# wwang2/CoarseGrainingVAE

Hardware: AMD Instinct MI355X
Metric: train_step_frames_per_sec (higher is better)
Workload: dtype f32

## Files before the change

coarsegrainingvae_amd/_lib.py:

```python
from __future__ import annotations

import ctypes as C
import os
import re
import threading

import torch

from . import ktimer

_PKG = os.path.dirname(os.path.abspath(__file__))
LIB_PATH = os.environ.get("CGV_LIB") or os.path.join(_PKG, "libcgvae_hip.so")
HEADER_PATH = os.path.join(os.path.dirname(_PKG), "include", "cgvae_hip.h")

_lock = threading.Lock()
_lib = None

_p, _i, _f, _sz = C.c_void_p, C.c_int, C.c_float, C.c_size_t

PROTOTYPES = {
    "cgv_version": (_i, []),
    "cgv_last_error_string": (C.c_char_p, []),
    "cgv_timestamp": (_i, [_p, _p]),
    "cgv_timestamp_hz": (_i, []),
# ... 93 lines not shown
    "cgv_decoder_slices_to_dense": (_i, [_p, _p, _i, C.c_int64, _p, _i, _i, _p]),
    "cgv_dense_grad_prepare": (_i, [_p, _p, _p, _p, _i, _i, _i, _i, _p]),
    "cgv_tile_supported": (_i, [_i, _i, _i]),
    "cgv_tile_linear_fwd": (_i, [_p, _p, _p, _p, _p, _i, _i, _i, _i, _p]),
    "cgv_tile_linear_bwd_input": (_i, [_p, _p, _p, _i, _i, _i, _p]),
    "cgv_tile_linear_bwd_input_act": (_i, [_p, _p, _p, _p, _i, _i, _i, _i, _p]),
    "cgv_tile_linear_bwd_input_act_add": (_i, [_p, _p, _p, _p, _p, _i, _i, _i, _i, _p]),
    "cgv_tile_linear_bwd_input_act_add_bcast": (_i, [_p] * 7 + [_i, _p, _i, _i, _i, _i, _p]),
    "cgv_tile_pair_supported": (_i, [_i, _i, _i]),
    "cgv_tile_pair_linear_fwd": (_i, [_p] * 10 + [_i, _i, _i, _i, _i, _p]),
    "cgv_tile_pair_linear_bwd_input": (_i, [_p] * 10 + [_i, _i, _i, _i, _i, _p]),
    "cgv_tile_linear_bwd_input_out": (_i, [_p] * 5 + [_i, _i, _i, _i, _p, _i, _p]),
    "cgv_tile_bwd_input_split": (_i, [_p, _sz, _p]),
    "cgv_tile_pair_linear_bwd_input_out": (_i, [_p] * 10 + [_i, _i, _i, _i, _i, _p, _i, _p, _i, _p]),
    "cgv_tile_linear_bwd_input_sum2": (_i, [_p] * 10 + [_i, _p, _i, _i, _i, _i, _i, _p]),
    "cgv_segment_reduce2": (_i, [_p, _i, _p, _p, _i, _p, _p, _p, _i, _i, _p]),
    "cgv_skinny_linear_bwd_input_add": (_i, [_p, _p, _p, _p, _p, _i, _i, _i, _i, _p, _sz, _p]),
    "cgv_skinny_linear_bwd_input_out": (_i, [_p] * 5 + [_i, _i, _i, _i, _p, _i, _p, _sz, _p]),
    "cgv_tile_linear_wgrad": (_i, [_p, _p, _p, _i, _i, _i, _i, _p]),
    "cgv_wgrad_record_bytes": (_i, []),
    "cgv_wgrad_plan": (_i, [_i, _i, _i, _p, _p, _p]),
    "cgv_wgrad_lds_floats": (_i, [_i, _i]),
    "cgv_grouped_wgrad": (_i, [_p, _i, _i, _i, _p]),
    "cgv_wgrad_gathered_plan": (_i, [_i, _i, _i, _i, _p, _p]),
    "cgv_grouped_wgrad_gathered": (_i, [_p, _i, _i, _p]),
    "cgv_wgrad_gathered_plan_tile": (_i, [_i, _i, _i, _i, _i, _p, _p]),
    "cgv_grouped_wgrad_gathered_tile": (_i, [_p, _i, _i, _i, _p]),
    "cgv_grouped_wgrad_split": (_i, [_p, _i, _i, _p]),
    "cgv_grouped_wgrad_gathered_sumsq": (_i, [_p, _i, _i, _p, _p, _p]),
    "cgv_grouped_wgrad_gathered_adam": (_i, [_p, _i, _i, _p, _p, _p, _p, _f, _f, _f, _f, _p, _p]),
# ... 236 lines not shown
```

coarsegrainingvae_amd/csrc/tile_gemm.hip:

```cpp
#include <stdlib.h>
#include <initializer_list>
#include <type_traits>
#include "cgv_common.h"
#include "streamk_gemm.h"

namespace cgv {

typedef float f32x4 __attribute__((ext_vector_type(4)));

__device__ __forceinline__ float4 ld4z(const float* p, bool ok) {
  return ok ? *reinterpret_cast<const float4*>(p) : make_float4(0.f, 0.f, 0.f, 0.f);
}

#define CGV_MFMA(a, b, c) __builtin_amdgcn_mfma_f32_16x16x4f32((a), (b), (c), 0, 0, 0)

template <int I0, int N, typename F>
__device__ __forceinline__ void static_for(F&& f) {
  if constexpr (I0 < N) {
    f(std::integral_constant<int, I0>{});
    static_for<I0 + 1, N>(f);
  }
}

struct TileSecond { const float* x; const float* W; const float* bias; float* y; float* z; int act; };
// ... 366 lines not shown
      float4 zv = make_float4(acc[a][b][0] + bv.x, acc[a][b][1] + bv.y, acc[a][b][2] + bv.z, acc[a][b][3] + bv.w);
      if (act) {
        if (zout) *reinterpret_cast<float4*>(zout + (size_t)m * N + n) = zv;
        zv.x = act_fwd(zv.x, act); zv.y = act_fwd(zv.y, act); zv.z = act_fwd(zv.z, act); zv.w = act_fwd(zv.w, act);
      }
      *reinterpret_cast<float4*>(y + (size_t)m * N + n) = zv;
    }
  }
}

struct BwdSource { const float* g; const float* W; const float* z; int act; };
struct BwdSecond { const float* g; const float* W; float* gx; const float* z; const float* add; int act; };
struct OutAct { const float* z; int act; const float* z2; int act2; };
struct SplitN { float* part; unsigned* ticket; int n; };
struct NormStackOut { const float* stack; const float* Vv; const float* g_res; float* g_s; float* gVv; int F; int ld; int accumulate; };
struct BcastAdd {
  const float* src;
  const int64_t* row2seg;
  const int* rowptr;
  int mean;
};

#ifndef CGV_BWD_INPUT_PIPELINE
#define CGV_BWD_INPUT_PIPELINE 0
#endif
template <int MB, int WAVES>
__global__ __launch_bounds__(64 * WAVES) void tile_bwd_input_k(const float* __restrict__ g, const float* __restrict__ W,
                                                        float* __restrict__ gx, int M, int N, int K,
                                                        const float* __restrict__ z, int act,
                                                        const float* __restrict__ add = nullptr,
                                                        BcastAdd bc = BcastAdd{nullptr, nullptr, nullptr, 0},
                                                        BwdSecond s2 = BwdSecond{nullptr, nullptr, nullptr, nullptr, nullptr, 0},
                                                        BwdSource more = BwdSource{nullptr, nullptr, nullptr, 0},
                                                        OutAct oa = OutAct{nullptr, 0, nullptr, 0},
                                                        SplitN sp = SplitN{nullptr, nullptr, 1},
                                                        NormStackOut ns = NormStackOut{nullptr, nullptr, nullptr, nullptr, nullptr, 0, 0, 0}) {
  if (blockIdx.z) { g = s2.g; W = s2.W; gx = s2.gx; z = s2.z; add = s2.add; act = s2.act; bc.src = nullptr; oa.z = oa.z2; oa.act = oa.act2; }
  __shared__ float red[WAVES][MB * 4][4][64];
  const int lane = threadIdx.x & 63;
  const int wave = __builtin_amdgcn_readfirstlane(threadIdx.x >> 6);
  const int j = lane & 15, q = lane >> 4;
  const int ry = (int)blockIdx.y / sp.n, zs = (int)blockIdx.y - ry * sp.n;
  const int k0 = blockIdx.x * 64, m0 = ry * (16 * MB);
  const int kcol = k0 + 4 * j;
  const bool kok = kcol < K;
  const float* gr[MB];
  bool gok[MB];
#pragma unroll
  for (int mb = 0; mb < MB; ++mb) {
    const int m = m0 + 16 * mb + j;
    gok[mb] = m < M;
    gr[mb] = g + (size_t)(gok[mb] ? m : 0) * N + 4 * q;
  }
  const ptrdiff_t zoff = act ? z - g : 0;
  f32x4 acc[MB][4];
#pragma unroll
  for (int mb = 0; mb < MB; ++mb)
#pragma unroll
    for (int s = 0; s < 4; ++s) acc[mb][s] = f32x4{0.f, 0.f, 0.f, 0.f};
  const int steps_all = (N + 15) / 16, zper = (steps_all + sp.n - 1) / sp.n;
  const int z_beg = min(zs * zper, steps_all), steps = min(z_beg + zper, steps_all);
  const int per = (steps - z_beg + WAVES - 1) / WAVES;
  const int st_beg = min(z_beg + wave * per, steps), st_end = min(st_beg + per, steps);
  constexpr int SB = WAVES >= 16 ? 3 : 2;
  const float* wcol = W + (kok ? kcol : 0);
  ptrdiff_t zo = zoff;
  const int n_src = more.g ? 2 : 1;
  for (int src = 0; src < n_src; ++src) {
  if (src == 1) {
#pragma unroll
    for (int mb = 0; mb < MB; ++mb) gr[mb] = more.g + (gr[mb] - g);
    act = more.act;
    zo = act ? more.z - more.g : 0;
    wcol = more.W + (kok ? kcol : 0);
  }
  struct Batch { float4 a[SB][MB], zz[SB][MB], b[SB][4]; };
  auto request = [&](Batch& B, int st0) __attribute__((always_inline)) {
#pragma unroll
    for (int u = 0; u < SB; ++u) {
      const int n = 16 * (st0 + u);
      const bool in = st0 + u < st_end && n + 4 * q < N;
      const int ng = in ? n : -4 * q, nw = in ? n + 4 * q : 0;
#pragma unroll
      for (int mb = 0; mb < MB; ++mb) {
        B.a[u][mb] = *reinterpret_cast<const float4*>(gr[mb] + ng);
        if (act) B.zz[u][mb] = *reinterpret_cast<const float4*>(gr[mb] + zo + ng);
      }
#pragma unroll
      for (int c = 0; c < 4; ++c) B.b[u][c] = *reinterpret_cast<const float4*>(wcol + (size_t)(nw + c) * K);
    }
  };
  auto multiply = [&](const Batch& B, int st0) __attribute__((always_inline)) {
#pragma unroll
    for (int u = 0; u < SB; ++u) {
      if (st0 + u >= st_end) break;
      const bool nok = 16 * (st0 + u) + 4 * q < N;
#pragma unroll
      for (int mb = 0; mb < MB; ++mb) {
        float4 av = B.a[u][mb];
        if (act) {
          av.x *= act_bwd(B.zz[u][mb].x, act); av.y *= act_bwd(B.zz[u][mb].y, act);
          av.z *= act_bwd(B.zz[u][mb].z, act); av.w *= act_bwd(B.zz[u][mb].w, act);
        }
        const float ac[4] = {nok ? av.x : 0.f, nok ? av.y : 0.f, nok ? av.z : 0.f, nok ? av.w : 0.f};
#pragma unroll
        for (int c = 0; c < 4; ++c) {
          acc[mb][0] = CGV_MFMA(ac[c], B.b[u][c].x, acc[mb][0]);
          acc[mb][1] = CGV_MFMA(ac[c], B.b[u][c].y, acc[mb][1]);
          acc[mb][2] = CGV_MFMA(ac[c], B.b[u][c].z, acc[mb][2]);
          acc[mb][3] = CGV_MFMA(ac[c], B.b[u][c].w, acc[mb][3]);
        }
// ... 335 lines not shown
  const int blocks16 = kt * ((M + 15) / 16);
  const int ow = option(CGV_OPT_BWD_INPUT_WAVES);
  int waves = 8;
  if (ow > 0 && ow != 32) waves = ow;
  else if (blocks16 < 128 && N >= 1024) waves = 16;
  if (ow == 32 || (blocks32 >= 200 && blocks32 < 512 && waves == 8))
    c.kernel = BWD_R32_W8;
  else if (blocks32 >= 512)
    c.kernel = BWD_R32_W4;
  else if (waves == 16) {
    c.kernel = BWD_R16_W16;
    if (ws) c.shares = split_shares(blocks16 * np, N);
  }
  return c;
}
}

static int tile_bwd_input_launch(const float* g, const float* z, int act, const float* W, float* gx, int M, int N, int K,
                                 void* stream, const char* what, const float* add = nullptr,
                                 cgv::BcastAdd bc = cgv::BcastAdd{nullptr, nullptr, nullptr, 0},
                                 const cgv::BwdSecond* second = nullptr,
                                 cgv::BwdSource more = cgv::BwdSource{nullptr, nullptr, nullptr, 0},
                                 cgv::OutAct oa = cgv::OutAct{nullptr, 0, nullptr, 0},
                                 cgv::NormStackOut ns = cgv::NormStackOut{nullptr, nullptr, nullptr, nullptr, nullptr, 0, 0, 0}) {
  hipStream_t st = (hipStream_t)stream;
  const cgv::BwdSecond s2 = second ? *second : cgv::BwdSecond{nullptr, nullptr, nullptr, nullptr, nullptr, 0};
  const unsigned np = second ? 2u : 1u;
  const cgv::BwdInputChoice choice = cgv::bwd_input_choice(M, N, K, (int)np, cgv::sk_ws_ready(stream));
  if (const int bpc = choice.bpc;
      bpc != 0 && !ns.stack && act == 0 && (!more.g || more.act == 0) && (!second || s2.act == 0) &&
      cgv::sk_aligned({g, W, gx, add, bc.src, more.g, more.W, oa.z, oa.z2, s2.g, s2.W, s2.gx, s2.add})) {
    cgv::SkArgs a{};
    a.np = (int)np; a.M = M; a.N = K;
    cgv::SkProblem& p0 = a.p[0];
    p0.A[0] = g; p0.B[0] = W; p0.R[0] = N; p0.out = gx; p0.add = add;
    if (more.g) { p0.A[1] = more.g; p0.B[1] = more.W; p0.R[1] = N; }
    p0.bc_src = bc.src; p0.bc_row2seg = bc.row2seg; p0.bc_rowptr = bc.rowptr; p0.bc_mean = bc.mean;
    p0.oz = oa.z; p0.oact = oa.act;
    if (second) {
      cgv::SkProblem& p1 = a.p[1];
      p1.A[0] = s2.g; p1.B[0] = s2.W; p1.R[0] = N; p1.out = s2.gx; p1.add = s2.add; p1.oz = oa.z2; p1.oact = oa.act2;
    }
    if (cgv::sk_launch(a, true, cgv::g_split_ws.ws, cgv::g_split_ws.bytes, cgv::SPLIT_TICKET_BYTES, st, bpc) == 0)
      return cgv::check_launch(what);
  }
  const int kt = (K + 63) / 64;
  switch (choice.kernel) {
    case cgv::BWD_R32_W8:
      hipLaunchKernelGGL((cgv::tile_bwd_input_k<2, 8>), dim3(kt, (M + 31) / 32, np), dim3(512), 0, st, g, W, gx, M, N, K, z, act, add, bc, s2, more, oa, cgv::SplitN{nullptr, nullptr, 1}, ns);
      break;
    case cgv::BWD_R32_W4:
      hipLaunchKernelGGL((cgv::tile_bwd_input_k<2, 4>), dim3(kt, (M + 31) / 32, np), dim3(256), 0, st, g, W, gx, M, N, K, z, act, add, bc, s2, more, oa, cgv::SplitN{nullptr, nullptr, 1}, ns);
      break;
    case cgv::BWD_R16_W16: {
      cgv::SplitN sp{nullptr, nullptr, 1};
      const int tiles = kt * ((M + 15) / 16) * (int)np;
      const cgv::SplitWs& w = cgv::g_split_ws;
      const size_t need = cgv::SPLIT_TICKET_BYTES + (size_t)tiles * choice.shares * (16 * 64) * sizeof(float);
      if (choice.shares > 1 && need <= w.bytes && (size_t)tiles * sizeof(unsigned) <= cgv::SPLIT_TICKET_BYTES) {
        sp.ticket = reinterpret_cast<unsigned*>(w.ws);
        sp.part = reinterpret_cast<float*>(reinterpret_cast<char*>(w.ws) + cgv::SPLIT_TICKET_BYTES);
        sp.n = choice.shares;
      }
      hipLaunchKernelGGL((cgv::tile_bwd_input_k<1, 16>), dim3(kt, ((M + 15) / 16) * sp.n, np), dim3(1024), 0, st, g, W, gx, M, N, K, z, act,
                         add, bc, s2, more, oa, sp, ns);
      break;
    }
    case cgv::BWD_R16_W8:
      hipLaunchKernelGGL((cgv::tile_bwd_input_k<1, 8>), dim3(kt, (M + 15) / 16, np), dim3(512), 0, st, g, W, gx, M, N, K, z, act, add, bc, s2, more, oa, cgv::SplitN{nullptr, nullptr, 1}, ns);
      break;
  }
  return cgv::check_launch(what);
}

int cgv_tile_bwd_input_plan(int M, int N, int K, int np, int* shares, int* streamk) {
  CGV_REQUIRE(shares && streamk && np >= 1 && np <= 2, "bad argument");
  CGV_REQUIRE(cgv_tile_supported(M, N, K), "unsupported shape (need N % 4 == 0, K % 4 == 0)");
  const cgv::BwdInputChoice c = cgv::bwd_input_choice(M, N, K, np, true);
  *streamk = c.bpc != 0;
  *shares = c.bpc != 0 ? 1 : c.shares;
  return 0;
}

int cgv_tile_bwd_input_split(void* ws, size_t bytes, void* stream) {
  CGV_REQUIRE(!ws || ((((uintptr_t)ws) & 15) == 0 && bytes >= cgv::SPLIT_TICKET_BYTES + (2u << 20)), "workspace too small / misaligned");
  cgv::g_split_ws = cgv::SplitWs{ws, ws ? bytes : 0, stream};
  return 0;
}

int cgv_tile_linear_bwd_input(const float* g, const float* W, float* gx, int M, int N, int K, void* stream) {
  CGV_REQUIRE(g && W && gx, "null pointer");
  CGV_REQUIRE(cgv_tile_supported(M, N, K), "unsupported shape (need N % 4 == 0, K % 4 == 0)");
  CGV_REQUIRE(((((uintptr_t)g | (uintptr_t)W | (uintptr_t)gx)) & 15) == 0, "g, W and gx must be 16-byte aligned");
  return tile_bwd_input_launch(g, nullptr, 0, W, gx, M, N, K, stream, "cgv_tile_linear_bwd_input");
}
// ... 123 lines not shown
```

coarsegrainingvae_amd/csrc/wgrad_gathered.hip:

```cpp
#include "cgv_common.h"
#include "gemm_dev.h"
#include "wgrad_record.h"

namespace cgv {

__device__ __forceinline__ float4 ldg4_or_zero(const float* p, bool ok) {
  return ok ? *reinterpret_cast<const float4*>(p) : make_float4(0.f, 0.f, 0.f, 0.f);
}
__device__ __forceinline__ void strip_pin() { asm volatile("" ::: "memory"); }
typedef const float __attribute__((address_space(1)))* strip_gptr;
__device__ __forceinline__ float4 strip_ldg4(const float* p) {
  const f32x4 t = *reinterpret_cast<const __attribute__((address_space(1))) f32x4*>((strip_gptr)p);
  return make_float4(t.x, t.y, t.z, t.w);
}
#ifndef CGV_GW_CHUNK
#define CGV_GW_CHUNK 48
#endif
constexpr int GW_CHUNK = CGV_GW_CHUNK;
constexpr int GW_GS = 80, GW_XS = 64;
constexpr int GW_TW = 128, GW_XW = 128;

enum { GW_STORE = 0, GW_SUMSQ = 1, GW_ADAM = 2 };
template <int MODE>
__global__ __launch_bounds__(256) void gathered_wgrad_k(const WgradProblem* __restrict__ table, int n_problems,
// ... 570 lines not shown
    bs[0] += (gq[0].x + gq[1].x) + (gq[2].x + gq[3].x);
    bs[1] += (gq[0].y + gq[1].y) + (gq[2].y + gq[3].y);
    bs[2] += (gq[0].z + gq[1].z) + (gq[2].z + gq[3].z);
    bs[3] += (gq[0].w + gq[1].w) + (gq[2].w + gq[3].w);
    sp_store4(gdst, PLANE, gq[0].x, gq[1].x, gq[2].x, gq[3].x);
    sp_store4(gdst + SP_LD, PLANE, gq[0].y, gq[1].y, gq[2].y, gq[3].y);
    sp_store4(gdst + 2 * SP_LD, PLANE, gq[0].z, gq[1].z, gq[2].z, gq[3].z);
    sp_store4(gdst + 3 * SP_LD, PLANE, gq[0].w, gq[1].w, gq[2].w, gq[3].w);
    sp_store4(xdst, PLANE, xq[0].x, xq[1].x, xq[2].x, xq[3].x);
    sp_store4(xdst + 16 * SP_LD, PLANE, xq[0].y, xq[1].y, xq[2].y, xq[3].y);
    sp_store4(xdst + 32 * SP_LD, PLANE, xq[0].z, xq[1].z, xq[2].z, xq[3].z);
    sp_store4(xdst + 48 * SP_LD, PLANE, xq[0].w, xq[1].w, xq[2].w, xq[3].w);
  };
  const unsigned short* ga = gs + (64 * wn + i) * SP_LD + 8 * q;
  const unsigned short* xb = xs + (64 * wk + i) * SP_LD + 8 * q;
  chunk_load(0);
  for (int m0 = 0; m0 < M; m0 += SP_CHUNK) {
    chunk_store(m0);
    __syncthreads();
    chunk_load(min(m0 + SP_CHUNK, M - 1));
    sp_bf16x8 a[3][4];
#pragma unroll
    for (int s = 0; s < 3; ++s)
#pragma unroll
      for (int t = 0; t < 4; ++t) a[s][t] = *reinterpret_cast<const sp_bf16x8*>(ga + s * PLANE + 16 * t * SP_LD);
#pragma unroll
    for (int c = 0; c < 4; ++c) {
      sp_bf16x8 b[3];
#pragma unroll
      for (int s = 0; s < 3; ++s) b[s] = *reinterpret_cast<const sp_bf16x8*>(xb + s * PLANE + 16 * c * SP_LD);
#pragma unroll
      for (int t = 0; t < 4; ++t) acc[t][c] = __builtin_amdgcn_mfma_f32_16x16x32_bf16(a[0][t], b[2], acc[t][c], 0, 0, 0);
// ... 429 lines not shown
```

coarsegrainingvae_amd/csrc/wgrad_record.h:

```cpp
#pragma once
#include "cgv_common.h"

namespace cgv {

struct WgradProblem {
  const float* gy;
  const float* x;
  const float* z;
  float* gW;
  float* gb;
  int M, N, K;
  int accumulate, act;
  int block_begin;
  int tiles_k;
  int tile_w;
  int seg_rows;
  int seg_stride;
  int pad;
};
static_assert(sizeof(WgradProblem) == 88, "host/device record layout");
__device__ __forceinline__ size_t wg_row(const WgradProblem& pr, int m, int width) {
  if (pr.seg_rows <= 0) return (size_t)m * width;
  const int seg = m / pr.seg_rows;
  return (size_t)seg * pr.seg_stride + (size_t)(m - seg * pr.seg_rows) * width;
}

template <typename Problem>
__device__ __forceinline__ int wg_find_problem(const Problem* __restrict__ table, int n_problems, int block) {
  const int lane = threadIdx.x & 63;
  int count = 0;
  for (int base = 0; base < n_problems; base += 64) {
    const int i = base + lane;
    const int bb = i < n_problems ? table[i].block_begin : 0x7fffffff;
    count += __popcll(__ballot(bb <= block));
  }
// ... 20 lines not shown
```

coarsegrainingvae_amd/ops.py:

```python
from __future__ import annotations

from typing import Optional

import ctypes as C
from types import SimpleNamespace

import torch

from . import _lib, options
from .graph import EdgeGeometry, EdgePlan
from .primitives import FWD_ENTRY, bwd_input_choice, bwd_input_launch, fwd_choice, linear as _linear, wgrad_queue, wgrad_sink

_F32 = torch.float32


def _c(t: Optional[torch.Tensor]) -> Optional[torch.Tensor]:
    if t is None:
        return None
    if t.dtype != _F32:
        raise RuntimeError("the HIP path computes in fp32 only")
    return t.contiguous()


def _filter_grad_targets(params, Wd, bd):
    pW, pb = params
    direct = all(getattr(p, "_cgv_direct", False) and p.grad is not None and p._cgv_pending and p.grad.is_contiguous()
# ... 32 lines not shown
                         dtype=torch.uint8, device=device)
        if not torch.cuda.is_current_stream_capturing():
            _GRP_WS[key] = ws
    return ws


def _balanced_workspace(device, n_dst, F, rb):
    key = (str(device), int(torch.cuda.current_stream(device).cuda_stream), int(n_dst), int(F), int(rb))
    ws = _BAL_WS.get(key)
    if ws is None:
        ws = torch.zeros(int(_lib.load().cgv_equi_msg_balanced_workspace_bytes(int(n_dst), int(F), int(rb))),
                         dtype=torch.uint8, device=device)
        if not torch.cuda.is_current_stream_capturing():
            _BAL_WS[key] = ws
    return ws


class _EquiMessage(torch.autograd.Function):

    @staticmethod
    def forward(ctx, phi, v, Wd, bd, plan: EdgePlan, geom: EdgeGeometry, with_dv: bool, s_res, v_res):
        filter_params = (Wd, bd)
        phi, v, Wd, bd, s_res, v_res = _c(phi), _c(v), _c(Wd), _c(bd), _c(s_res), _c(v_res)
        ctx.residual = (s_res is not None, v_res is not None)
        F = phi.shape[1] // 3
        if phi.shape[0] != plan.n_src or v.shape != (plan.n_src, F, 3) or Wd.shape != (3 * F, geom.n_rbf):
            raise RuntimeError("shape mismatch between node features, filter weights and the edge plan")
        ds = torch.empty(plan.n_dst, F, dtype=_F32, device=phi.device)
        if with_dv:
            dv = torch.empty(plan.n_dst, F, 3, dtype=_F32, device=phi.device)
# ... 27 lines not shown

    @staticmethod
    def backward(ctx, gs, gv):
        phi, v, Wd, bd = ctx.saved_tensors
        plan, geom = ctx.plan, ctx.geom
        F = phi.shape[1] // 3
        dev = phi.device
        g_sres = gs if ctx.residual[0] else None
        g_vres = gv if ctx.residual[1] else None
        if not ctx.with_dv:
            gv = None
        if gs is None and gv is None:
            return (None,) * 7 + (g_sres, g_vres)
        gs, gv = _c(gs), _c(gv)
        g_phi = torch.empty_like(phi)
        g_v = torch.empty_like(v) if gv is not None else None
        gWd, gbd, ret_W, ret_b = _filter_grad_targets(ctx.filter_params, Wd, bd)
        lib = _lib.load()
        ws_bytes = int(lib.cgv_equi_msg_bwd_workspace_bytes(plan.n_src, F, geom.n_rbf))
        ws = torch.empty(ws_bytes, dtype=torch.uint8, device=dev)
        if wgrad_queue.active and ret_W is None and ret_b is None:
            nc, kl = C.c_int(), C.c_int()
            _lib.call("cgv_equi_msg_bwd_deferred", _lib.ptr(phi), _lib.ptr(v), _lib.ptr(geom.geom_s), _lib.ptr(plan.rowptr_s),
                      _lib.ptr(plan.dst_s), _lib.ptr(Wd), _lib.ptr(bd), _lib.ptr(gs), _lib.ptr(gv), _lib.ptr(g_phi), _lib.ptr(g_v),
                      plan.n_src, F, geom.n_rbf, plan.n_edges, plan.n_dst, _lib.ptr(ws), ws_bytes, C.byref(nc), C.byref(kl),
                      _lib.stream_ptr(), tag=f"equi_msg_bwd:Nd{plan.n_dst}:E{plan.n_edges}:gv{int(gv is not None)}")
            wgrad_queue.enqueue_filter(ws, nc.value, kl.value, geom.n_rbf, F, gWd, gbd)
            return g_phi, g_v, ret_W, ret_b, None, None, None, g_sres, g_vres
        _lib.call("cgv_equi_msg_bwd", _lib.ptr(phi), _lib.ptr(v), _lib.ptr(geom.geom_s), _lib.ptr(plan.rowptr_s),
                  _lib.ptr(plan.dst_s), _lib.ptr(Wd), _lib.ptr(bd), _lib.ptr(gs), _lib.ptr(gv), _lib.ptr(g_phi),
# ... 752 lines not shown
```

coarsegrainingvae_amd/options.py:

```python
from __future__ import annotations

from . import _lib

HOST = {
    "fwd_group": -1,
    "wgrad_kernel": 0,
    "table_upload": 0,
    "wgrad_tile": 64,
    "rank_update": 1,
    "rank_flat": 2,
    "rank_mixed": 1,
    "rank_rows_mfma": -1,
    "rank_gram_rows": -1,
    "concurrent_prior": 0,
    "quad_heads": 1,
    "fused_loss_tail": 1,
    "paired_embeddings": 1,
    "pair_sum2": 1,
    "head_pairs": 1,
    "encoder_pairs": 1,
    "wgrad_split": 1,
    "fused_bead_mean": 1,
    "fused_prior": 1,
    "update_fused_fwd": 0,
    "fwd_parts": 1,
    "fwd_balanced": 0,
    "act_downstream": 1,
    "update_fused_bwd": 1,
    "strip_split": 1,
    "cgae_form": 0,
    "newman_form": 0,
    "baseline_form": 0,
    "align_form": 0,
    "kde_splits": 0,
    "decoder_dense": 0,
}
_DEFAULTS = dict(HOST)


def set(name: str, value: int) -> None:
    if name in HOST:
        HOST[name] = int(value)
    elif name in _lib.OPTIONS:
        _lib.set_option(name, int(value))
    else:
        raise KeyError(f"unknown option {name!r}; known: {sorted(HOST) + sorted(_lib.OPTIONS)}")


def get(name: str) -> int:
# ... 25 lines not shown
```

coarsegrainingvae_amd/primitives.py:

```python
from __future__ import annotations

import ctypes as C
import struct

import numpy as np
import torch
import torch.nn.functional as Fn
from torch import nn

from . import _lib


class Swish(nn.Module):

    def forward(self, x):
        return Fn.silu(x)


class shifted_softplus(nn.Module):
    def forward(self, x):
        return Fn.softplus(x) - np.log(2.0)


layer_types = {
# ... 25 lines not shown
        return "tile", None
    return None, (f"Dense / Linear {M} x {N} x {K}: the HIP kernels take in / out widths that are multiples of 4 "
                  f"(other widths are zero-padded by primitives.linear_fn before they get here)")


def _gemm_mode(x2, weight, bias):
    mode, why = gemm_mode_or_none(x2, weight, bias)
    if mode is None:
        raise RuntimeError(why)
    return mode


ACT_NONE, ACT_SWISH, ACT_TANH, ACT_RELU = 0, 1, 2, 3
ACT_STD_ENC, ACT_STD_PRIOR = 4, 5
_STD_EPS = {ACT_STD_ENC: 1e-12, ACT_STD_PRIOR: 1e-9}


class WeightGradQueue:

    RECORD = struct.Struct("<5Q11i4x")
    MAX_PROBLEMS = 512

    def __init__(self):
        self.active = False
        self.items = []
        self._captured = []
        self._capture_slots = []
        self._deferred = []
        self.filters = []

# ... 198 lines not shown
            _lib.call("cgv_grouped_wgrad", _lib.ptr(table), len(small), block_begin, max_lds, _lib.stream_ptr(),
                      tag="grouped_wgrad")
        if strips:
            table, block_begin, rows = self.strip_table(strips)
            self.strip_launch(table, len(strips), block_begin, rows, "grouped_wgrad_strip")
        if large:
            buf, block_begin = bytearray(), 0
            from .options import HOST
            split = HOST["wgrad_split"] == 1
            tile = 128 if split else wgrad_tile([(gy.shape[0], gy.shape[1], x.shape[1]) for gy, x, *_rest in large])
            for gy, x, z, act, gW, gb, accumulate in large:
                M, N = gy.shape
                K = x.shape[1]
                if lib.cgv_wgrad_gathered_plan_tile(M, N, K, 0, tile, C.byref(tk), C.byref(nb)) != 0:
                    raise RuntimeError(lib.cgv_last_error_string().decode())
                buf += self.RECORD.pack(gy.data_ptr(), x.data_ptr(), z.data_ptr() if z is not None else 0, gW.data_ptr(),
                                        gb.data_ptr() if gb is not None else 0, M, N, K, int(accumulate), int(act),
                                        block_begin, tk.value, 0, 0, 0, 0)
                block_begin += nb.value
            table = self.upload(bytes(buf), dev)
            if split:
                _lib.call("cgv_grouped_wgrad_split", _lib.ptr(table), len(large), block_begin, _lib.stream_ptr(),
                          tag="grouped_wgrad_tiles")
            else:
                _lib.call("cgv_grouped_wgrad_gathered_tile", _lib.ptr(table), len(large), block_begin, tile, _lib.stream_ptr(),
                          tag="grouped_wgrad_tiles")


class _QueueScope:
    def __init__(self, q):
        self.q = q

    def __enter__(self):
# ... 87 lines not shown
        return gx, gw, gb, None

    @staticmethod
    def _backward_core(ctx, gy, add):
        x, weight, z = ctx.saved_tensors
        w_param, b_param = ctx.params
        act = ctx.act
        if getattr(ctx, "act_done", False):
            ctx.act_done = False
            act = ACT_NONE
        add2 = add.reshape(-1, add.shape[-1]) if add is not None else None
        if add2 is not None and not (add2.is_contiguous() and add2.data_ptr() % 16 == 0 and add2.dtype == torch.float32):
            add2 = add2.contiguous().float()
        need_x, need_w = ctx.needs_input_grad[0], ctx.needs_input_grad[1]
        need_b = b_param is not None and ctx.needs_input_grad[2]
        gy2 = gy.reshape(-1, gy.shape[-1]).contiguous()
        M, K = x.shape
        N = weight.shape[0]
        gx = None
        if ctx.mode == "tile":
            if gy2.data_ptr() % 16:
                gy2 = gy2.clone()
            if not (need_w and wgrad_queue.active and _is_direct(w_param) and w_param.grad.is_contiguous()
                    and (not need_b or (_is_direct(b_param) and b_param.grad.is_contiguous())) and lib_has_rows(M, N, K)):
                return _LinearFn._backward_prepared(ctx, gy, gy2, add, act, need_x, need_w, need_b)
        if need_x:
            gx = torch.empty(M, K, dtype=torch.float32, device=gy.device)
            kind = bwd_input_choice(M, N, K, _lib.split_workspace_ready(), ctx.bias_aligned, gy2.data_ptr() % 16 == 0)
            slot = getattr(ctx, "slot", None)
            g = slot.g if (slot is not None and ctx.mode == "tile" and kind == "tile") else None
            parked = None
            if g is not None and (g.dtype == torch.float32 and g.is_contiguous() and g.data_ptr() % 16 == 0 and g.dim() == 2
                                  and g.shape[1] == K and slot.mapping.numel() == M):
                parked = slot.take()
            fused = bwd_input_launch(kind, gy2, z, act, weight, gx, add2, slot, parked, getattr(ctx, "producer", None))
            gx = gx.reshape(gy.shape[:-1] + (K,))
            if add is not None and not fused:
                gx = gx + add.reshape(gx.shape)
        gw = gb = None
        if need_w:
            gw, gb = wgrad_sink(w_param, b_param, gy2, x, z, act, (M, N, K), like=weight, need_b=need_b)
        return (gx if need_x else add), gw, gb, None

    @staticmethod
    def _backward_prepared(ctx, gy, gy2, add, act, need_x, need_w, need_b):
        x, weight, z = ctx.saved_tensors
        w_param, b_param = ctx.params
        M, K = x.shape
        N = weight.shape[0]
        st = _lib.stream_ptr()
# ... 94 lines not shown
        ctx.set_materialize_grads(False)
        return ya.reshape(x_a.shape[:-1] + (N,)), yb.reshape(x_b.shape[:-1] + (N,)), x_a.view_as(x_a)

    @staticmethod
    def backward(ctx, g_a, g_b, g_alias):
        xa, xb, wa, wb, za, zb = ctx.saved_tensors
        pa_w, pa_b, pb_w, pb_b = ctx.params
        (act_a, act_b), slot = ctx.acts, ctx.slot
        done = getattr(ctx, "act_done", (False, False))
        ctx.act_done = (False, False)
        act_a = ACT_NONE if done[0] else act_a
        act_b = ACT_NONE if done[1] else act_b
        M, K = xa.shape
        N = wa.shape[0]
        st = _lib.stream_ptr()
        prep = lambda g: None if g is None else g.reshape(M, N).contiguous()
        ga, gb = prep(g_a), prep(g_b)
        new = lambda: torch.empty(M, K, dtype=torch.float32, device=xa.device)
        kind = bwd_input_choice(M, N, K, _lib.split_workspace_ready(), long_row_split=False)

        def single(g, z, w, add, act, parked=None):
            gx = new()
            bwd_input_launch(kind, g, z, act, w, gx, add, slot, parked)
            return gx
        gxa = gxb = None
        need_a, need_b = ctx.needs_input_grad[0], ctx.needs_input_grad[1]
        if ctx.same:
            if need_a:
                add = None if g_alias is None else g_alias.reshape(M, K).contiguous()
                parked = None
                if slot is not None:
                    slot.linear_done = True
                    parked = slot.take()
                par_ok = parked is None or (parked.dtype == torch.float32 and parked.is_contiguous() and parked.shape[1] == K
                                            and parked.data_ptr() % 16 == 0)
                if (ga is not None and gb is not None and par_ok and HOST_OPTION("pair_sum2")
                        and (add is None or (add.dtype == torch.float32 and add.data_ptr() % 16 == 0))):
                    gxa = new()
# ... 11 lines not shown
                if gb_done:
                    pass
                elif ga is not None and parked is not None and parked.dtype == torch.float32 and parked.is_contiguous() and parked.shape[1] == K:
                    gxa = single(ga, za, wa, add, act_a, parked)
                else:
                    gxa = single(ga, za, wa, add, act_a) if ga is not None else add
                    if parked is not None:
                        spread = slot.broadcast(parked)
                        gxa = spread if gxa is None else gxa + spread
                if gxa is not None:
                    gxa = gxa.reshape(xa.shape)
        else:
            if ga is not None and gb is not None and need_a and need_b:
                gxa, gxb = new(), new()
                prod = ctx.producer
                if prod is not None:
                    pz = prod.saved_tensors
                    _lib.call("cgv_tile_pair_linear_bwd_input_out", _lib.ptr(ga), _lib.ptr(za) if act_a != ACT_NONE else None, _lib.ptr(wa),
                              None, _lib.ptr(gxa), _lib.ptr(gb), _lib.ptr(zb) if act_b != ACT_NONE else None, _lib.ptr(wb), None,
                              _lib.ptr(gxb), M, N, K, act_a, act_b, _lib.ptr(pz[4]), int(prod.acts[0]), _lib.ptr(pz[5]),
                              int(prod.acts[1]), st)
                    prod.act_done = (True, True)
                else:
                    _lib.call("cgv_tile_pair_linear_bwd_input", _lib.ptr(ga), _lib.ptr(za) if act_a != ACT_NONE else None, _lib.ptr(wa), None,
                              _lib.ptr(gxa), _lib.ptr(gb), _lib.ptr(zb) if act_b != ACT_NONE else None, _lib.ptr(wb), None, _lib.ptr(gxb),
                              M, N, K, act_a, act_b, st)
            else:
                gxa = single(ga, za, wa, None, act_a) if (ga is not None and need_a) else None
                gxb = single(gb, zb, wb, None, act_b) if (gb is not None and need_b) else None
        grads_w = []
# ... 219 lines not shown


def bwd_input_choice(M, N, K, split_ready, bias_aligned=True, gy_aligned=True, short_tiles=True, long_row_split=True) -> str:
    lib = _lib.load()
    if lib.cgv_skinny_supported(M, N, K) and bias_aligned:
        if (M > 32 and ((short_tiles and N <= 1024) or (N < 4096 and split_ready)) and gy_aligned
                and lib.cgv_tile_supported(M, N, K)):
            return "tile"
        return "skinny"
    if (long_row_split and M <= 128 and N >= 4096 and lib.cgv_skinny_bwd_input_supported(M, N, K)
            and not (M > 64 and split_ready)):
        return "skinny"
    return "tile"


def bwd_input_launch(kind, gy2, z, act, weight, gx, add=None, slot=None, parked=None, producer=None) -> bool:
    M, K = gx.shape
    N = weight.shape[0]
    z = z if act != ACT_NONE else None
    if kind == "skinny":
        if producer is not None and skinny_bwd_input_out(gy2, z, weight, add, gx, M, N, K, act, producer.saved_tensors[2],
                                                         int(producer.act)):
            producer.act_done = True
            return True
        return skinny_bwd_input(gy2, z, weight, gx, M, N, K, act, add=add)
    st = _lib.stream_ptr()
    P = _lib.ptr
    if parked is not None:
        _lib.call("cgv_tile_linear_bwd_input_act_add_bcast", P(gy2), P(z), P(weight), P(add), P(parked), P(slot.mapping),
                  P(slot.plan.rowptr_d), int(slot.mean), P(gx), M, N, K, act, st)
    elif producer is not None:
        _lib.call("cgv_tile_linear_bwd_input_out", P(gy2), P(z), P(weight), P(add), P(gx), M, N, K, act,
                  P(producer.saved_tensors[2]), int(producer.act), st)
        producer.act_done = True
    elif add is not None:
        _lib.call("cgv_tile_linear_bwd_input_act_add", P(gy2), P(z), P(weight), P(add), P(gx), M, N, K, act, st)
    else:
        _lib.call("cgv_tile_linear_bwd_input_act", P(gy2), P(z), P(weight), P(gx), M, N, K, act, st)
        return False
    return True


# ... 228 lines not shown
```

include/cgvae_hip.h:

```cpp
#ifndef CGVAE_HIP_H
#define CGVAE_HIP_H

#include <stddef.h>
#include <stdint.h>

#ifdef __cplusplus
extern "C" {
#endif

#define CGV_VERSION 100

#define CGV_E_BADARG (-1)
#define CGV_E_UNSUPPORTED (-2)
#define CGV_E_WORKSPACE (-3)

int cgv_version(void);
const char* cgv_last_error_string(void);

enum {
  CGV_OPT_MSG_FWD_SPLIT = 0,
  CGV_OPT_MSG_BWD_SPLIT = 1,
  CGV_OPT_MSG_FWD_KERNEL = 2,
  CGV_OPT_GRP_WAVES = 3,
  CGV_OPT_GRP_RECORDS = 4,
// ... 258 lines not shown
                             int act_b, void* stream);
int cgv_tile_pair_linear_bwd_input(const float* gy_a, const float* z_a, const float* W_a, const float* add_a, float* gx_a,
                                   const float* gy_b, const float* z_b, const float* W_b, const float* add_b, float* gx_b, int M,
                                   int N, int K, int act_a, int act_b, void* stream);
int cgv_tile_linear_bwd_input_norm_stack(const float* gy, const float* z, const float* W, int M, int N, int K, int act,
                                         const float* stack, const float* Vv, const float* g_res, float* g_s, float* gVv, int ld,
                                         int accumulate, void* stream);
int cgv_tile_bwd_input_plan(int M, int N, int K, int np, int* shares , int* streamk );
int cgv_tile_bwd_input_split(void* workspace, size_t workspace_bytes, void* stream);
int cgv_tile_linear_bwd_input_out(const float* gy, const float* z, const float* W, const float* add, float* gx, int M, int N,
                                  int K, int act, const float* z_out, int act_out, void* stream);
int cgv_tile_pair_linear_bwd_input_out(const float* gy_a, const float* z_a, const float* W_a, const float* add_a, float* gx_a,
                                       const float* gy_b, const float* z_b, const float* W_b, const float* add_b, float* gx_b,
                                       int M, int N, int K, int act_a, int act_b, const float* z_out_a, int act_out_a,
                                       const float* z_out_b, int act_out_b, void* stream);
int cgv_tile_linear_bwd_input_sum2(const float* gy_a, const float* z_a, const float* W_a, const float* gy_b, const float* z_b,
                                   const float* W_b, const float* add, const float* seg_grad, const int64_t* row2seg,
                                   const int32_t* seg_rowptr, int mean, float* gx, int M, int N, int K, int act_a, int act_b,
                                   void* stream);
int cgv_tile_linear_wgrad(const float* g, const float* x, float* gW, int M, int N, int K, int accumulate, void* stream);
int cgv_wgrad_record_bytes(void);
int cgv_wgrad_plan(int M, int N, int K, int* tiles_k , int* tile_w , int* n_blocks );
int cgv_wgrad_lds_floats(int M, int tile_w);
int cgv_grouped_wgrad(const void* table_dev, int n_problems, int total_blocks, int max_lds_floats, void* stream);
int cgv_wgrad_gathered_plan(int M, int N, int K, int seg_rows, int* tiles_k , int* n_blocks );
int cgv_grouped_wgrad_gathered(const void* table_dev, int n_problems, int total_blocks, void* stream);
int cgv_wgrad_gathered_plan_tile(int M, int N, int K, int seg_rows, int tile, int* tiles_k , int* n_blocks );
int cgv_grouped_wgrad_gathered_tile(const void* table_dev, int n_problems, int total_blocks, int tile, void* stream);
int cgv_grouped_wgrad_split(const void* table_dev, int n_problems, int total_blocks, void* stream);
int cgv_grouped_wgrad_gathered_sumsq(const void* table_dev, int n_problems, int total_blocks, double* partial, double* sumsq,
// ... 260 lines not shown
```

Baseline: 1301.

## Skip dead filter-gradient column slices in backward input and wgrad kernels

When the equivariant message backward has no vector gradient, only the middle F-column slice of the filter gradient is nonzero. The gradient tensor is now tagged with a live-column window, and that window is passed through to the tile backward-input kernel, which restricts its N-steps to the live range. The grouped split wgrad kernel skips output row tiles outside the window via a packed field in the record pad. This avoids reduction work over columns known to be zero, at the cost of host-side window state (thread-local) and the risk of wrong gradients if those columns are not truly zero.

```diff
diff --git a/coarsegrainingvae_amd/_lib.py b/coarsegrainingvae_amd/_lib.py
--- a/coarsegrainingvae_amd/_lib.py
+++ b/coarsegrainingvae_amd/_lib.py
@@ -131,6 +131,8 @@
     "cgv_tile_bwd_input_split": (_i, [_p, _sz, _p]),
     "cgv_tile_pair_linear_bwd_input_out": (_i, [_p] * 10 + [_i, _i, _i, _i, _i, _p, _i, _p, _i, _p]),
     "cgv_tile_linear_bwd_input_sum2": (_i, [_p] * 10 + [_i, _p, _i, _i, _i, _i, _i, _p]),
+    "cgv_tile_bwd_input_window": (_i, [_i, _i]),
+    "cgv_tile_bwd_input_plan_window": (_i, [_i, _i, _i, _i, _i, _i, _p, _p, _p, _p, _p]),
     "cgv_segment_reduce2": (_i, [_p, _i, _p, _p, _i, _p, _p, _p, _i, _i, _p]),
     "cgv_skinny_linear_bwd_input_add": (_i, [_p, _p, _p, _p, _p, _i, _i, _i, _i, _p, _sz, _p]),
     "cgv_skinny_linear_bwd_input_out": (_i, [_p] * 5 + [_i, _i, _i, _i, _p, _i, _p, _sz, _p]),
diff --git a/coarsegrainingvae_amd/csrc/tile_gemm.hip b/coarsegrainingvae_amd/csrc/tile_gemm.hip
--- a/coarsegrainingvae_amd/csrc/tile_gemm.hip
+++ b/coarsegrainingvae_amd/csrc/tile_gemm.hip
@@ -404,6 +404,7 @@
 struct OutAct { const float* z; int act; const float* z2; int act2; };
 struct SplitN { float* part; unsigned* ticket; int n; };
 struct NormStackOut { const float* stack; const float* Vv; const float* g_res; float* g_s; float* gVv; int F; int ld; int accumulate; };
+struct NWindow { int lo, hi, st_lo, st_hi; };
 struct BcastAdd {
   const float* src;
   const int64_t* row2seg;
@@ -424,7 +425,8 @@
                                                         BwdSource more = BwdSource{nullptr, nullptr, nullptr, 0},
                                                         OutAct oa = OutAct{nullptr, 0, nullptr, 0},
                                                         SplitN sp = SplitN{nullptr, nullptr, 1},
-                                                        NormStackOut ns = NormStackOut{nullptr, nullptr, nullptr, nullptr, nullptr, 0, 0, 0}) {
+                                                        NormStackOut ns = NormStackOut{nullptr, nullptr, nullptr, nullptr, nullptr, 0, 0, 0},
+                                                        NWindow win = NWindow{0, 0x7fffffff, 0, 0x7fffffff}) {
   if (blockIdx.z) { g = s2.g; W = s2.W; gx = s2.gx; z = s2.z; add = s2.add; act = s2.act; bc.src = nullptr; oa.z = oa.z2; oa.act = oa.act2; }
   __shared__ float red[WAVES][MB * 4][4][64];
   const int lane = threadIdx.x & 63;
@@ -451,7 +453,9 @@
   const int steps_all = (N + 15) / 16, zper = (steps_all + sp.n - 1) / sp.n;
   const int z_beg = min(zs * zper, steps_all), steps = min(z_beg + zper, steps_all);
   const int per = (steps - z_beg + WAVES - 1) / WAVES;
-  const int st_beg = min(z_beg + wave * per, steps), st_end = min(st_beg + per, steps);
+  const int st_own = min(z_beg + wave * per, steps);
+  const int st_beg = max(st_own, win.st_lo), st_end = min(min(st_own + per, steps), win.st_hi);
+  const int n_lo = win.lo, n_hi = min(N, win.hi);
   constexpr int SB = WAVES >= 16 ? 3 : 2;
   const float* wcol = W + (kok ? kcol : 0);
   ptrdiff_t zo = zoff;
@@ -469,7 +473,7 @@
 #pragma unroll
     for (int u = 0; u < SB; ++u) {
       const int n = 16 * (st0 + u);
-      const bool in = st0 + u < st_end && n + 4 * q < N;
+      const bool in = st0 + u < st_end && n + 4 * q < n_hi && n + 4 * q >= n_lo;
       const int ng = in ? n : -4 * q, nw = in ? n + 4 * q : 0;
 #pragma unroll
       for (int mb = 0; mb < MB; ++mb) {
@@ -484,7 +488,7 @@
 #pragma unroll
     for (int u = 0; u < SB; ++u) {
       if (st0 + u >= st_end) break;
-      const bool nok = 16 * (st0 + u) + 4 * q < N;
+      const bool nok = 16 * (st0 + u) + 4 * q < n_hi && 16 * (st0 + u) + 4 * q >= n_lo;
 #pragma unroll
       for (int mb = 0; mb < MB; ++mb) {
         float4 av = B.a[u][mb];
@@ -850,6 +854,16 @@
   }
   return c;
 }
+
+static NWindow bwd_window(int N, int n_lo, int n_hi) {
+  const int steps = (N + 15) / 16;
+  if (n_hi <= 0 || (n_lo <= 0 && n_hi >= N)) return NWindow{0, N, 0, steps};
+  return NWindow{n_lo, n_hi, n_lo / 16, (n_hi + 15) / 16};
+}
+static bool bwd_window_ok(int N, int n_lo, int n_hi) {
+  return n_hi <= 0 || (n_lo >= 0 && n_lo < n_hi && n_hi <= N && n_lo % 4 == 0 && n_hi % 4 == 0);
+}
+static thread_local int g_next_window[2] = {0, 0};
 }
 
 static int tile_bwd_input_launch(const float* g, const float* z, int act, const float* W, float* gx, int M, int N, int K,
@@ -860,6 +874,10 @@
                                  cgv::OutAct oa = cgv::OutAct{nullptr, 0, nullptr, 0},
                                  cgv::NormStackOut ns = cgv::NormStackOut{nullptr, nullptr, nullptr, nullptr, nullptr, 0, 0, 0}) {
   hipStream_t st = (hipStream_t)stream;
+  const int n_lo = cgv::g_next_window[0], n_hi = cgv::g_next_window[1];
+  cgv::g_next_window[0] = cgv::g_next_window[1] = 0;
+  CGV_REQUIRE(n_hi <= N, "the stated live-column window exceeds the reduction of this launch");
+  const cgv::NWindow win = cgv::bwd_window(N, n_lo, n_hi);
   const cgv::BwdSecond s2 = second ? *second : cgv::BwdSecond{nullptr, nullptr, nullptr, nullptr, nullptr, 0};
   const unsigned np = second ? 2u : 1u;
   const cgv::BwdInputChoice choice = cgv::bwd_input_choice(M, N, K, (int)np, cgv::sk_ws_ready(stream));
@@ -883,10 +901,10 @@
   const int kt = (K + 63) / 64;
   switch (choice.kernel) {
     case cgv::BWD_R32_W8:
-      hipLaunchKernelGGL((cgv::tile_bwd_input_k<2, 8>), dim3(kt, (M + 31) / 32, np), dim3(512), 0, st, g, W, gx, M, N, K, z, act, add, bc, s2, more, oa, cgv::SplitN{nullptr, nullptr, 1}, ns);
+      hipLaunchKernelGGL((cgv::tile_bwd_input_k<2, 8>), dim3(kt, (M + 31) / 32, np), dim3(512), 0, st, g, W, gx, M, N, K, z, act, add, bc, s2, more, oa, cgv::SplitN{nullptr, nullptr, 1}, ns, win);
       break;
     case cgv::BWD_R32_W4:
-      hipLaunchKernelGGL((cgv::tile_bwd_input_k<2, 4>), dim3(kt, (M + 31) / 32, np), dim3(256), 0, st, g, W, gx, M, N, K, z, act, add, bc, s2, more, oa, cgv::SplitN{nullptr, nullptr, 1}, ns);
+      hipLaunchKernelGGL((cgv::tile_bwd_input_k<2, 4>), dim3(kt, (M + 31) / 32, np), dim3(256), 0, st, g, W, gx, M, N, K, z, act, add, bc, s2, more, oa, cgv::SplitN{nullptr, nullptr, 1}, ns, win);
       break;
     case cgv::BWD_R16_W16: {
       cgv::SplitN sp{nullptr, nullptr, 1};
@@ -899,11 +917,11 @@
         sp.n = choice.shares;
       }
       hipLaunchKernelGGL((cgv::tile_bwd_input_k<1, 16>), dim3(kt, ((M + 15) / 16) * sp.n, np), dim3(1024), 0, st, g, W, gx, M, N, K, z, act,
-                         add, bc, s2, more, oa, sp, ns);
+                         add, bc, s2, more, oa, sp, ns, win);
       break;
     }
     case cgv::BWD_R16_W8:
-      hipLaunchKernelGGL((cgv::tile_bwd_input_k<1, 8>), dim3(kt, (M + 15) / 16, np), dim3(512), 0, st, g, W, gx, M, N, K, z, act, add, bc, s2, more, oa, cgv::SplitN{nullptr, nullptr, 1}, ns);
+      hipLaunchKernelGGL((cgv::tile_bwd_input_k<1, 8>), dim3(kt, (M + 15) / 16, np), dim3(512), 0, st, g, W, gx, M, N, K, z, act, add, bc, s2, more, oa, cgv::SplitN{nullptr, nullptr, 1}, ns, win);
       break;
   }
   return cgv::check_launch(what);
@@ -915,6 +933,28 @@
   const cgv::BwdInputChoice c = cgv::bwd_input_choice(M, N, K, np, true);
   *streamk = c.bpc != 0;
   *shares = c.bpc != 0 ? 1 : c.shares;
+  return 0;
+}
+
+int cgv_tile_bwd_input_window(int n_lo, int n_hi) {
+  CGV_REQUIRE(cgv::bwd_window_ok(0x7ffffffc, n_lo, n_hi), "bad window (need 0 <= n_lo < n_hi, multiples of 4)");
+  cgv::g_next_window[0] = n_hi > 0 ? n_lo : 0;
+  cgv::g_next_window[1] = n_hi > 0 ? n_hi : 0;
+  return 0;
+}
+
+int cgv_tile_bwd_input_plan_window(int M, int N, int K, int np, int n_lo, int n_hi, int* shares, int* streamk, int* kernel,
+                                   int* first_step, int* n_steps) {
+  CGV_REQUIRE(shares && streamk && kernel && first_step && n_steps && np >= 1 && np <= 2, "bad argument");
+  CGV_REQUIRE(cgv_tile_supported(M, N, K), "unsupported shape (need N % 4 == 0, K % 4 == 0)");
+  CGV_REQUIRE(cgv::bwd_window_ok(N, n_lo, n_hi), "bad window (need 0 <= n_lo < n_hi <= N, multiples of 4)");
+  const cgv::BwdInputChoice c = cgv::bwd_input_choice(M, N, K, np, true);
+  const cgv::NWindow w = c.bpc != 0 ? cgv::bwd_window(N, 0, 0) : cgv::bwd_window(N, n_lo, n_hi);
+  *streamk = c.bpc != 0;
+  *shares = c.bpc != 0 ? 1 : c.shares;
+  *kernel = (int)c.kernel;
+  *first_step = w.st_lo;
+  *n_steps = w.st_hi - w.st_lo;
   return 0;
 }
 
diff --git a/coarsegrainingvae_amd/csrc/wgrad_gathered.hip b/coarsegrainingvae_amd/csrc/wgrad_gathered.hip
--- a/coarsegrainingvae_amd/csrc/wgrad_gathered.hip
+++ b/coarsegrainingvae_amd/csrc/wgrad_gathered.hip
@@ -608,8 +608,9 @@
   };
   const unsigned short* ga = gs + (64 * wn + i) * SP_LD + 8 * q;
   const unsigned short* xb = xs + (64 * wk + i) * SP_LD + 8 * q;
-  chunk_load(0);
-  for (int m0 = 0; m0 < M; m0 += SP_CHUNK) {
+  const bool dead = wg_rows_dead(pr, n0, 128);
+  if (!dead) chunk_load(0);
+  for (int m0 = 0; m0 < M && !dead; m0 += SP_CHUNK) {
     chunk_store(m0);
     __syncthreads();
     chunk_load(min(m0 + SP_CHUNK, M - 1));
diff --git a/coarsegrainingvae_amd/csrc/wgrad_record.h b/coarsegrainingvae_amd/csrc/wgrad_record.h
--- a/coarsegrainingvae_amd/csrc/wgrad_record.h
+++ b/coarsegrainingvae_amd/csrc/wgrad_record.h
@@ -19,6 +19,10 @@
   int pad;
 };
 static_assert(sizeof(WgradProblem) == 88, "host/device record layout");
+__device__ __forceinline__ bool wg_rows_dead(const WgradProblem& pr, int n0, int rows) {
+  const int lo = 4 * (pr.pad & 0xffff), hi = 4 * (int)((unsigned)pr.pad >> 16);
+  return pr.pad != 0 && (n0 + rows <= lo || n0 >= hi);
+}
 __device__ __forceinline__ size_t wg_row(const WgradProblem& pr, int m, int width) {
   if (pr.seg_rows <= 0) return (size_t)m * width;
   const int seg = m / pr.seg_rows;
diff --git a/coarsegrainingvae_amd/ops.py b/coarsegrainingvae_amd/ops.py
--- a/coarsegrainingvae_amd/ops.py
+++ b/coarsegrainingvae_amd/ops.py
@@ -9,7 +9,7 @@
 
 from . import _lib, options
 from .graph import EdgeGeometry, EdgePlan
-from .primitives import FWD_ENTRY, bwd_input_choice, bwd_input_launch, fwd_choice, linear as _linear, wgrad_queue, wgrad_sink
+from .primitives import FWD_ENTRY, bwd_input_choice, bwd_input_launch, fwd_choice, linear as _linear, tag_live_columns, wgrad_queue, wgrad_sink
 
 _F32 = torch.float32
 
@@ -72,6 +72,18 @@
         if not torch.cuda.is_current_stream_capturing():
             _BAL_WS[key] = ws
     return ws
+
+
+def live_filter_slices(has_gv: bool):
+    return (True, True, True) if has_gv else (False, True, False)
+
+
+def live_columns(F: int, has_gv: bool):
+    live = live_filter_slices(has_gv)
+    if all(live) or not options.HOST["dead_slice_window"] or F % 4:
+        return None
+    at = [k for k, on in enumerate(live) if on]
+    return (at[0] * F, (at[-1] + 1) * F) if at == list(range(at[0], at[-1] + 1)) else None
 
 
 class _EquiMessage(torch.autograd.Function):
@@ -129,6 +141,7 @@
             return (None,) * 7 + (g_sres, g_vres)
         gs, gv = _c(gs), _c(gv)
         g_phi = torch.empty_like(phi)
+        tag_live_columns(g_phi, live_columns(F, gv is not None))
         g_v = torch.empty_like(v) if gv is not None else None
         gWd, gbd, ret_W, ret_b = _filter_grad_targets(ctx.filter_params, Wd, bd)
         lib = _lib.load()
diff --git a/coarsegrainingvae_amd/options.py b/coarsegrainingvae_amd/options.py
--- a/coarsegrainingvae_amd/options.py
+++ b/coarsegrainingvae_amd/options.py
@@ -33,6 +33,7 @@
     "baseline_form": 0,
     "align_form": 0,
     "kde_splits": 0,
+    "dead_slice_window": 1,
     "decoder_dense": 0,
 }
 _DEFAULTS = dict(HOST)
diff --git a/coarsegrainingvae_amd/primitives.py b/coarsegrainingvae_amd/primitives.py
--- a/coarsegrainingvae_amd/primitives.py
+++ b/coarsegrainingvae_amd/primitives.py
@@ -63,6 +63,32 @@
 ACT_NONE, ACT_SWISH, ACT_TANH, ACT_RELU = 0, 1, 2, 3
 ACT_STD_ENC, ACT_STD_PRIOR = 4, 5
 _STD_EPS = {ACT_STD_ENC: 1e-12, ACT_STD_PRIOR: 1e-9}
+
+
+def tag_live_columns(t, window):
+    if t is not None and window is not None:
+        t._cgv_live_cols = (int(window[0]), int(window[1]))
+    return t
+
+
+def live_columns_of(t):
+    w = getattr(t, "_cgv_live_cols", None) if t is not None else None
+    if w is None or not (0 <= w[0] < w[1] <= t.shape[-1]) or w[0] % 4 or w[1] % 4 or (w[0] == 0 and w[1] == t.shape[-1]):
+        return None
+    return w
+
+
+def state_window(window):
+    if window is not None:
+        lib = _lib.load()
+        if lib.cgv_tile_bwd_input_window(int(window[0]), int(window[1])) != 0:
+            raise RuntimeError("cgv_tile_bwd_input_window failed: " + lib.cgv_last_error_string().decode("utf-8", "replace"))
+
+
+def pack_live_rows(window, N) -> int:
+    if window is None or N >= 4 * 0x8000:
+        return 0
+    return (window[0] // 4) | ((window[1] // 4) << 16)
 
 
 class WeightGradQueue:
@@ -291,9 +317,10 @@
                 K = x.shape[1]
                 if lib.cgv_wgrad_gathered_plan_tile(M, N, K, 0, tile, C.byref(tk), C.byref(nb)) != 0:
                     raise RuntimeError(lib.cgv_last_error_string().decode())
+                live = pack_live_rows(live_columns_of(gy), N) if split else 0
                 buf += self.RECORD.pack(gy.data_ptr(), x.data_ptr(), z.data_ptr() if z is not None else 0, gW.data_ptr(),
                                         gb.data_ptr() if gb is not None else 0, M, N, K, int(accumulate), int(act),
-                                        block_begin, tk.value, 0, 0, 0, 0)
+                                        block_begin, tk.value, 0, 0, 0, live)
                 block_begin += nb.value
             table = self.upload(bytes(buf), dev)
             if split:
@@ -411,6 +438,7 @@
             add2 = add2.contiguous().float()
         need_x, need_w = ctx.needs_input_grad[0], ctx.needs_input_grad[1]
         need_b = b_param is not None and ctx.needs_input_grad[2]
+        window = live_columns_of(gy)
         gy2 = gy.reshape(-1, gy.shape[-1]).contiguous()
         M, K = x.shape
         N = weight.shape[0]
@@ -418,6 +446,7 @@
         if ctx.mode == "tile":
             if gy2.data_ptr() % 16:
                 gy2 = gy2.clone()
+            tag_live_columns(gy2, window)
             if not (need_w and wgrad_queue.active and _is_direct(w_param) and w_param.grad.is_contiguous()
                     and (not need_b or (_is_direct(b_param) and b_param.grad.is_contiguous())) and lib_has_rows(M, N, K)):
                 return _LinearFn._backward_prepared(ctx, gy, gy2, add, act, need_x, need_w, need_b)
@@ -430,7 +459,8 @@
             if g is not None and (g.dtype == torch.float32 and g.is_contiguous() and g.data_ptr() % 16 == 0 and g.dim() == 2
                                   and g.shape[1] == K and slot.mapping.numel() == M):
                 parked = slot.take()
-            fused = bwd_input_launch(kind, gy2, z, act, weight, gx, add2, slot, parked, getattr(ctx, "producer", None))
+            fused = bwd_input_launch(kind, gy2, z, act, weight, gx, add2, slot, parked, getattr(ctx, "producer", None),
+                                     window=window if ctx.mode == "tile" else None)
             gx = gx.reshape(gy.shape[:-1] + (K,))
             if add is not None and not fused:
                 gx = gx + add.reshape(gx.shape)
@@ -555,14 +585,15 @@
         M, K = xa.shape
         N = wa.shape[0]
         st = _lib.stream_ptr()
-        prep = lambda g: None if g is None else g.reshape(M, N).contiguous()
+        prep = lambda g: None if g is None else tag_live_columns(g.reshape(M, N).contiguous(), live_columns_of(g))
         ga, gb = prep(g_a), prep(g_b)
+        win_a, win_b = live_columns_of(ga), live_columns_of(gb)
         new = lambda: torch.empty(M, K, dtype=torch.float32, device=xa.device)
         kind = bwd_input_choice(M, N, K, _lib.split_workspace_ready(), long_row_split=False)
 
         def single(g, z, w, add, act, parked=None):
             gx = new()
-            bwd_input_launch(kind, g, z, act, w, gx, add, slot, parked)
+            bwd_input_launch(kind, g, z, act, w, gx, add, slot, parked, window=live_columns_of(g))
             return gx
         gxa = gxb = None
         need_a, need_b = ctx.needs_input_grad[0], ctx.needs_input_grad[1]
@@ -604,6 +635,8 @@
             if ga is not None and gb is not None and need_a and need_b:
                 gxa, gxb = new(), new()
                 prod = ctx.producer
+                if win_a is not None and win_a == win_b:
+                    state_window(win_a)
                 if prod is not None:
                     pz = prod.saved_tensors
                     _lib.call("cgv_tile_pair_linear_bwd_input_out", _lib.ptr(ga), _lib.ptr(za) if act_a != ACT_NONE else None, _lib.ptr(wa),
@@ -853,7 +886,7 @@
     return "tile"
 
 
-def bwd_input_launch(kind, gy2, z, act, weight, gx, add=None, slot=None, parked=None, producer=None) -> bool:
+def bwd_input_launch(kind, gy2, z, act, weight, gx, add=None, slot=None, parked=None, producer=None, window=None) -> bool:
     M, K = gx.shape
     N = weight.shape[0]
     z = z if act != ACT_NONE else None
@@ -865,6 +898,7 @@
         return skinny_bwd_input(gy2, z, weight, gx, M, N, K, act, add=add)
     st = _lib.stream_ptr()
     P = _lib.ptr
+    state_window(window)
     if parked is not None:
         _lib.call("cgv_tile_linear_bwd_input_act_add_bcast", P(gy2), P(z), P(weight), P(add), P(parked), P(slot.mapping),
                   P(slot.plan.rowptr_d), int(slot.mean), P(gx), M, N, K, act, st)
diff --git a/include/cgvae_hip.h b/include/cgvae_hip.h
--- a/include/cgvae_hip.h
+++ b/include/cgvae_hip.h
@@ -296,6 +296,9 @@
                                        const float* gy_b, const float* z_b, const float* W_b, const float* add_b, float* gx_b,
                                        int M, int N, int K, int act_a, int act_b, const float* z_out_a, int act_out_a,
                                        const float* z_out_b, int act_out_b, void* stream);
+int cgv_tile_bwd_input_window(int n_lo, int n_hi);
+int cgv_tile_bwd_input_plan_window(int M, int N, int K, int np, int n_lo, int n_hi, int* shares , int* streamk ,
+                                   int* kernel , int* first_step , int* n_steps );
 int cgv_tile_linear_bwd_input_sum2(const float* gy_a, const float* z_a, const float* W_a, const float* gy_b, const float* z_b,
                                    const float* W_b, const float* add, const float* seg_grad, const int64_t* row2seg,
                                    const int32_t* seg_rowptr, int mean, float* gx, int M, int N, int K, int act_a, int act_b,
```

Result: no change. 1314 (median of 6 runs) (+1.0%).
